# tanwanirahul/surreal

Hardware: AMD Instinct MI355X
Metric: PPO learner env-steps/sec/node (GAE+update) at 1/2/4/8 GPUs; % HBM roofline (higher is better)
Workload: dtype f32; 1 GPU; C3: synthetic PPO learner batch, reference PPO defaults (LSTM 100, horizon 5, heads 300x200, n_step 25, adapt, z-filter, 10/10 epochs), SawyerLift state dims (obs 42, act 8), 1024 segments split over 1 GPU(s) (1024 per GPU); segments_per_gpu=1024, n_step=25, env_steps_per_learn_per_gpu=25600, global_segments=1024, parallelism=single, epochs_run_last=10, ppo_mode=adapt, launch=hipGraph replay

## Files before the change

### include/surreal_mi.h

```cpp
#ifndef SURREAL_MI_H
#define SURREAL_MI_H

#include <stdint.h>

#ifdef __cplusplus
extern "C" {
#endif

#define SMI_OK            0
#define SMI_E_ARG        -1
#define SMI_E_NOFIT      -2
#define SMI_E_LAUNCH     -3

int         smi_version(void);
const char* smi_last_error(void);

const char* smi_last_launch(void);

int64_t smi_workspace_bytes(void);
int     smi_set_workspace(void* dev_ptr, int64_t bytes);
typedef struct smi_context smi_context;
smi_context* smi_context_create(void* workspace, int64_t bytes);
int          smi_context_make_current(smi_context* ctx);
int          smi_context_destroy(smi_context* ctx);
// ... 223 lines not shown
int64_t smi_ppo_rnn_xbuf_floats(int obs_dim, int rnn_hidden, int h1, int h2, int act_dim,
                                int critic_h1, int critic_h2, int pix_c, int pix_h, int pix_w,
                                int cnn_feat, int rnn_layer);
int64_t smi_lstm_param_count(int in_dim, int hidden);
int smi_ppo_rnn_phase(const smi_ppo_rnn_args* args, int phase, int epoch, void* stream);

int smi_lstm_forward(const float* xproj, const float* w_hh, const float* b_hh,
                     const float* h0, const float* c0, int S, int B, int H,
                     float* hbuf, float* cbuf, float* gates_act, void* stream);
int smi_lstm_backward(const float* dh, const float* gates_act, const float* cbuf,
                      const float* w_hh, int S, int B, int H, float* dgates, void* stream);
int smi_lstm_forward_x(const float* x, int64_t ldx, int din, const float* w_ih,
                       const float* b_ih, const float* w_hh, const float* b_hh,
                       const float* h0, const float* c0, int S, int B, int H, float* hbuf,
                       float* cbuf, float* gates_act, float* xproj_scratch, void* stream);

int64_t smi_cnn_param_count(int C, int H, int W, int F);
int64_t smi_cnn_scratch_bytes(int64_t rows, int C, int H, int W, int F);
int smi_cnn_backward_prefetch(int C, int H, int W);
int smi_cnn_forward(const float* params, const uint8_t* pix, const uint8_t* pix_next, int64_t B,
                    int64_t T, int64_t rows, int C, int H, int W, int F, float* a1, float* a2,
                    float* feat, int64_t ldf, void* stream);
int smi_cnn_backward(const float* params, const uint8_t* pix, const uint8_t* pix_next, int64_t B,
                     int64_t T, int64_t rows, int C, int H, int W, int F, const float* a1,
                     const float* a2, const float* dz, int64_t lddz, float* grad, void* scratch,
                     int64_t scratch_bytes, void* stream);

int smi_zfilter_accumulate(const float* sum_in, const float* sumsq_in, int dim, float rows,
                           float* running_sum, float* running_sumsq, float* count,
                           void* stream);
// ... 113 lines not shown
```

### surreal_amd/_lib.py

```python
import contextlib
import threading
import ctypes
import gc
import os

import torch

HERE = os.path.dirname(os.path.abspath(__file__))
_VARIANT = os.environ.get('SMI_LIB_VARIANT')
LIB_PATH = os.path.join(HERE, 'libsurreal_mi.so' if not _VARIANT else f'libsurreal_mi_{_VARIANT}.so')

c_int, c_i64, c_f32, c_f64, c_vp = ctypes.c_int, ctypes.c_int64, ctypes.c_float, ctypes.c_double, ctypes.c_void_p
P = ctypes.c_void_p

HYP_CLIP_EPS, HYP_BETA, HYP_LR_ACTOR, HYP_LR_CRITIC, HYP_CLIP_LO, HYP_CLIP_HI, HYP_COUNT = range(7)
ST_NAMES = ['_surr_loss', '_clip_surr_loss', '_kl_loss_adapt', '_entropy', '_pol_kl',
            'grad_norm_actor', '_val_loss', '_val_explained_var', 'grad_norm_critic',
            '_avg_return_targ', '_avg_log_sig', '_avg_behave_likelihood', '_avg_is_weight',
            '_ref_behave_diff', 'epochs_run', '_pol_kl_adapt']
ST_COUNT = len(ST_NAMES)
ST = {n: i for i, n in enumerate(ST_NAMES)}


class PPOArgs(ctypes.Structure):
# ... 172 lines not shown
    'smi_clock_probe': (c_int, [P, ctypes.c_longlong, P, P]),
    'smi_clock_probe_stop': (c_int, [P, c_int, P]),
    'smi_ppo_rnn_scratch_bytes': (c_i64, [c_int] * 15),
    'smi_ppo_rnn_xbuf_floats': (c_i64, [c_int] * 12),
    'smi_cnn_param_count': (c_i64, [c_int] * 4),
    'smi_cnn_scratch_bytes': (c_i64, [c_i64] + [c_int] * 4),
    'smi_cnn_backward_prefetch': (c_int, [c_int] * 3),
    'smi_cnn_forward': (c_int, [P, P, P, c_i64, c_i64, c_i64] + [c_int] * 4 + [P, P, P, c_i64, P]),
    'smi_cnn_backward': (c_int, [P, P, P, c_i64, c_i64, c_i64] + [c_int] * 4 +
                         [P, P, P, c_i64, P, P, c_i64, P]),
    'smi_ppo_rnn_phase': (c_int, [ctypes.POINTER(RNNArgs), c_int, c_int, P]),
    'smi_lstm_forward': (c_int, [P, P, P, P, P, c_int, c_int, c_int, P, P, P, P]),
    'smi_lstm_backward': (c_int, [P, P, P, P, c_int, c_int, c_int, P, P]),
    'smi_lstm_forward_x': (c_int, [P, c_i64, c_int, P, P, P, P, P, P, c_int, c_int, c_int,
                                   P, P, P, P, P]),
}

_lib = None


def lib():
    global _lib
    if _lib is None:
        if not os.path.exists(LIB_PATH):
            raise RuntimeError('libsurreal_mi.so not built: run `python -c "import __graft_entry__ as '
                               'g; g.build()"` (no CPU fallback exists)')
        L = ctypes.CDLL(LIB_PATH)
        for name, (res, args) in _SIGS.items():
            fn = getattr(L, name)
            fn.restype = res
# ... 87 lines not shown
```

### surreal_amd/csrc/capi.hip

```cpp
#include <stdio.h>
#include <string.h>
#include <atomic>
#include "smi_device.hpp"
#include "smi_internal.hpp"
#include "rnn_layout.hpp"

namespace smi {

static thread_local char g_err[512] = "";
static thread_local const char* g_last_launch = "";

int set_error(int code, const char* msg) {
  snprintf(g_err, sizeof(g_err), "%s", msg);
  return code;
}

int check_launch(const char* what) {
  g_last_launch = what;
  const hipError_t e = hipGetLastError();
  if (e != hipSuccess) {
    snprintf(g_err, sizeof(g_err), "%s: %s", what, hipGetErrorString(e));
    return -(int)e;
  }
  return SMI_OK;
// ... 789 lines not shown
                       float* gates_act, float* xproj_scratch, void* stream) {
  REQUIRE(x && w_ih && b_ih && w_hh && b_hh && h0 && c0 && hbuf && S >= 0 && B >= 0 && H >= 1 &&
          din >= 1 && ldx >= din, "lstm_forward_x: bad args");
  const hipStream_t st = SMI_STREAM(stream);
  const int rf = launch_lstm_fwd_x(x, ldx, din, w_ih, b_ih, w_hh, b_hh, h0, c0, S, B, H, hbuf, cbuf,
                                   gates_act, st, nullptr, 0);
  if (rf != SMI_E_NOFIT) return rf;
  REQUIRE(xproj_scratch, "lstm_forward_x: the unfused form needs xproj_scratch [S][B][4H]");
  const int rc = launch_linear_fwd(x, ldx, S * B, din, w_ih, din, b_ih, 4 * H, ACT_NONE,
                                   xproj_scratch, 4 * H, st, nullptr);
  if (rc) return rc;
  return launch_lstm_fwd(xproj_scratch, w_hh, b_hh, h0, c0, S, B, H, hbuf, cbuf, gates_act, st,
                         nullptr);
}

int smi_lstm_backward(const float* dh, const float* gates_act, const float* cbuf,
                      const float* w_hh, int S, int B, int H, float* dgates, void* stream) {
  REQUIRE(dh && gates_act && cbuf && w_hh && dgates && S >= 0 && B >= 0 && H >= 1,
          "lstm_backward: bad args");
  return launch_lstm_bwd(dh, gates_act, cbuf, w_hh, S, B, H, dgates, SMI_STREAM(stream), nullptr);
}

}
```

### surreal_amd/csrc/lstm_mfma.hip

```cpp
#include "smi_device.hpp"
#include "smi_internal.hpp"
#include "lstm_cell.hpp"

namespace smi {

constexpr int LR = 16;
#ifdef SMI_PROF
__device__ unsigned long long g_lstm_ticks[8];
#endif

__host__ __device__ inline int lstm_ld(int k) {
  int l = round4(k);
  if ((l & 7) != 4) l += 4;
  return l;
}

__host__ __device__ inline int lstm_q(int K) { return (((K + 3) >> 2) + 3) & ~3; }

constexpr int MAXUT = 4;
__global__ void __launch_bounds__(kWG)
lstm_fwd_kernel(LstmFwdArgs a) {
  if (a.skip && a.skip[0] != 0) return;
  const int keepS = a.keep > 0 ? a.keep : a.S;
  extern __shared__ __attribute__((aligned(16))) float sm[];
// ... 252 lines not shown
__device__ __forceinline__ void load_row_v(const float* r, int n, float* dst) {
  static_assert(N % 4 == 0 && (V == 4 || V == 2), "vector rows");
#pragma unroll
  for (int k = 0; k < N; k += V) {
    const float* src = k < n ? r + k : g_lstm_zero4;
    if constexpr (V == 4) {
      const float4 v = *reinterpret_cast<const float4*>(src);
      dst[k] = v.x; dst[k + 1] = v.y; dst[k + 2] = v.z; dst[k + 3] = v.w;
    } else {
      const float2 v = *reinterpret_cast<const float2*>(src);
      dst[k] = v.x; dst[k + 1] = v.y;
    }
  }
}

template <int KP, int KX, bool VF = false>
__global__ void __launch_bounds__(kWG8)
lstm_fwd_r4_kernel(LstmFwdArgs a) {
  if (a.skip && a.skip[0] != 0) return;
  LSTM_T0();
  const int keepS = a.keep > 0 ? a.keep : a.S;
  constexpr int KXS = KX > 0 ? KX : 8;
  __shared__ __attribute__((aligned(16))) float hS[2][LR4 * KP];
  __shared__ __attribute__((aligned(16))) float xS[2][LR4 * KXS];
  __shared__ float pre[LR4][4 * KP];
  const int H = a.H, B = a.B, G4 = 4 * H;
  const int tid = threadIdx.x, lane = tid & 63, wave = tid >> 6;
  const int r0 = blockIdx.x * LR4;
  const int64_t BH = (int64_t)B * H;
  const int col = wave * 64 + lane;
  const bool cact = wave * 64 < G4;
  const int colc = col < G4 ? col : G4 - 1;
  float w[KP];
  float wx[KXS];
  float bh = a.b_hh[colc];
  if constexpr (KX > 0) bh += a.b_ih[colc];
  if constexpr (VF) {
    load_row_v<KP, 4>(a.w_hh + (int64_t)colc * H, H, w);
    if constexpr (KX > 0) load_row_v<KX, 2>(a.w_ih + (int64_t)colc * a.din, a.din, wx);
  } else {
    load_row<KP>(a.w_hh + (int64_t)colc * H, H, w);
    if constexpr (KX > 0) load_row<KX>(a.w_ih + (int64_t)colc * a.din, a.din, wx);
  }
  const int xr = tid / KXS, xk = tid - (tid / KXS) * KXS;
  const bool xown = KX > 0 && tid < LR4 * KXS;
  const int64_t xoff0 = (int64_t)min(r0 + xr, B - 1) * a.ldx + min(xk, a.din - 1);
  const bool xval = xk < a.din;
  auto xload = [&](int t) -> float { return a.x[(int64_t)t * B * a.ldx + xoff0]; };
  float xnext = 0.f, x0 = 0.f;
  if constexpr (KX > 0) {
    x0 = xload(0);
    xnext = xload(a.S > 1 ? 1 : 0);
// ... 237 lines not shown
    __syncthreads();
  }
}

static int device_cus() {
  static int cus = 0;
  if (!cus) {
    int dev = 0;
    (void)hipGetDevice(&dev);
    if (hipDeviceGetAttribute(&cus, hipDeviceAttributeMultiprocessorCount, dev) != hipSuccess || cus < 1)
      cus = 256;
  }
  return cus;
}
static bool lstm_valu(int B, int H) { return H >= 1 && H <= 128 && B <= device_cus(); }

#ifdef SMI_PROF
extern "C" int smi_lstm_phase_ticks(unsigned long long* out ) {
  if (hipMemcpyFromSymbol(out, HIP_SYMBOL(g_lstm_ticks), sizeof(g_lstm_ticks)) != hipSuccess)
    return SMI_E_LAUNCH;
  static const unsigned long long zero[8] = {0, 0, 0, 0, 0, 0, 0, 0};
  return hipMemcpyToSymbol(HIP_SYMBOL(g_lstm_ticks), zero, sizeof(zero)) == hipSuccess ? SMI_OK
                                                                                        : SMI_E_LAUNCH;
}
#endif

int64_t lstm_fwd_lds(int H) { return (int64_t)2 * LR * lstm_ld(4 * lstm_q(H)) * 4; }
int64_t lstm_bwd_lds(int H) { return (int64_t)2 * LR * lstm_ld(4 * H) * 4; }

static bool r4_vf(const LstmFwdArgs& a, bool fused_x) {
  auto al = [](const void* p, uintptr_t m) { return (reinterpret_cast<uintptr_t>(p) & m) == 0; };
  if (a.H % 4 != 0 || !al(a.w_hh, 15)) return false;
  return !fused_x || (a.din % 2 == 0 && a.din >= 2 && al(a.w_ih, 7));
}

int launch_lstm_fwd(const float* xproj, const float* w_hh, const float* b_hh, const float* h0,
                    const float* c0, int S, int B, int H, float* hbuf, float* cbuf, float* gates,
                    hipStream_t st, const int* skip, int keep) {
  if (B <= 0 || S < 0) return SMI_OK;
  if (H < 1 || H > 256) return set_error(SMI_E_ARG, "lstm: hidden size must be in [1, 256]");
  LstmFwdArgs a{xproj, w_hh, b_hh, h0, c0, S, B, H, hbuf, cbuf, gates, skip};
  a.keep = keep;
  const int kslot = ktime_begin(st);
  struct End { int s; hipStream_t st; double f;
               ~End() { ktime_end(s, KT_LSTM_FWD, f, st); } } end_{kslot, st, 8.0 * B * H * (double)H * S};
  if (lstm_valu(B, H)) return check_launch(lstm_v_fwd(a, 0, st));
  if (H <= 128) {
    const dim3 g4((B + LR4 - 1) / LR4);
    const bool vf = r4_vf(a, false);
#define SMI_R4F(KP_)                                                                        \
    do {                                                                                    \
      if (vf) {                                                                             \
        hipLaunchKernelGGL((lstm_fwd_r4_kernel<KP_, 0, true>), g4, dim3(kWG8), 0, st, a);   \
        return check_launch("lstm_fwd_r4_kernel<" #KP_ ",0,vf>");                           \
      } else {                                                                              \
        hipLaunchKernelGGL((lstm_fwd_r4_kernel<KP_, 0>), g4, dim3(kWG8), 0, st, a);         \
        return check_launch("lstm_fwd_r4_kernel<" #KP_ ",0>");                              \
      }                                                                                     \
    } while (0)
    if (H <= 32) SMI_R4F(32);
    else if (H <= 64) SMI_R4F(64);
    else if (H <= 104) SMI_R4F(104);
    else SMI_R4F(128);
#undef SMI_R4F
  }
  const size_t lds = (size_t)lstm_fwd_lds(H);
  const dim3 grid((B + LR - 1) / LR);
  allow_lds(lstm_fwd_kernel, lds);
  hipLaunchKernelGGL(lstm_fwd_kernel, grid, dim3(kWG), lds, st, a);
  return check_launch("lstm_fwd_kernel<4>");
}

int launch_lstm_fwd_x(const float* x, int64_t ldx, int din, const float* w_ih, const float* b_ih,
                      const float* w_hh, const float* b_hh, const float* h0, const float* c0,
                      int S, int B, int H, float* hbuf, float* cbuf, float* gates,
                      hipStream_t st, const int* skip, int keep) {
  if (B <= 0 || S <= 0) return SMI_OK;
  if (din < 1 || din > 64 || H < 1 || H > 104) return SMI_E_NOFIT;
  const bool valu = lstm_valu(B, H);
  if (valu && lstm_fwd_v_lds(S, din <= 48 ? 48 : 64, (4 * H + 63) & ~63) > kVxMax)
    return SMI_E_NOFIT;
  LstmFwdArgs a{nullptr, w_hh, b_hh, h0, c0, S, B, H, hbuf, cbuf, gates, skip,
                x, ldx, din, w_ih, b_ih, keep};
  const int kslot = ktime_begin(st);
  struct End { int s; hipStream_t st; double f;
               ~End() { ktime_end(s, KT_LSTM_FWD, f, st); } } end_{
      kslot, st, 8.0 * B * H * (double)(H + din) * S};
  if (valu) return check_launch(lstm_v_fwd(a, din <= 48 ? 48 : 64, st));
  const dim3 g4((B + LR4 - 1) / LR4);
  const bool vf = r4_vf(a, true);
#define SMI_R4X(KP_, KX_)                                                                     \
  do {                                                                                        \
    if (vf) {                                                                                 \
      hipLaunchKernelGGL((lstm_fwd_r4_kernel<KP_, KX_, true>), g4, dim3(kWG8), 0, st, a);     \
      return check_launch("lstm_fwd_r4_kernel<" #KP_ "," #KX_ ",vf>");                        \
    } else {                                                                                  \
      hipLaunchKernelGGL((lstm_fwd_r4_kernel<KP_, KX_>), g4, dim3(kWG8), 0, st, a);           \
      return check_launch("lstm_fwd_r4_kernel<" #KP_ "," #KX_ ">");                           \
    }                                                                                         \
  } while (0)
  if (din <= 48) {
    if (H <= 64) SMI_R4X(64, 48);
    else SMI_R4X(104, 48);
  } else {
    if (H <= 64) SMI_R4X(64, 64);
    else SMI_R4X(104, 64);
  }
#undef SMI_R4X
// ... 64 lines not shown
```

### surreal_amd/csrc/ppo_rnn.hip

```cpp
#include "smi_device.hpp"
#include "smi_internal.hpp"
#include "dw_plan.hpp"
#include "pol_rows.hpp"
#include "lstm_cell.hpp"
#include "rnn_layout.hpp"
#include "rnn_kernels.hpp"

namespace smi {

struct Head {
  const float* P; MlpLayout L; int in, h1, h2, out, tanh_out;
};

static bool head_fused(const Head& h, const float* X, int64_t ldx) {
  return head_fused_ok(h.in, ldx, h.h1, h.h2, h.out, X, h.P + h.L.fW1, h.P + h.L.fW2,
                       h.P + h.L.fW3);
}

struct HeadFwdOpts {
  const int* skip = nullptr;
  float* wT = nullptr;
  bool keep_act = true;
  const float* vret = nullptr;
  float* vgrad = nullptr;
// ... 55 lines not shown
  RC_CHECK(launch_linear_bwd_dx(dZ, h.out, M, h.out, h.P + L.fW3, h.h2, h.h2, HA2, h.h2, dH2,
                                h.h2, st, skip));
  RC_CHECK(launch_linear_bwd_dw(dH2, h.h2, M, h.h2, HA1, h.h1, h.h1, G + L.fW2, h.h1, G + L.fb2,
                                0, st, skip));
  RC_CHECK(launch_linear_bwd_dx(dH2, h.h2, M, h.h2, h.P + L.fW2, h.h1, h.h1, HA1, h.h1, dH1,
                                h.h1, st, skip));
  RC_CHECK(launch_linear_bwd_dw(dH1, h.h1, M, h.h1, X, ldx, h.in, G + L.fW1, h.in, G + L.fb1, 0,
                                st, skip));
  if (dxn <= 0) return SMI_OK;
  return launch_linear_bwd_dx(dH1, h.h1, M, h.h1, h.P + L.fW1 + dx0, h.in, dxn, dxmask, ldm, dXout,
                              dxn, st, skip);
}

static int lstm_forward(const RnnDims& d, const float* P, const float* X, int S, const float* h0,
                        const float* c0, const RnnScratch& s, bool keep, hipStream_t st,
                        const int* skip, int keep_steps = 0) {
  const int64_t BH = (int64_t)d.B * d.H;
  for (int l = 0; l < d.L; ++l) {
    const LstmP lp = lstm_layer(d, P, l);
    const float* Xl = l == 0 ? X : hbuf_of(d, s, l - 1) + BH;
    const int64_t ldx = l == 0 ? d.ldx : d.H;
    const int din = l == 0 ? d.Din : d.H;
    float* hb = hbuf_of(d, s, l);
    float* cb = keep ? cbuf_of(d, s, l) : nullptr;
    float* gt = keep ? gates_of(d, s, l) : nullptr;
    const int rf = launch_lstm_fwd_x(Xl, ldx, din, lp.Wih, lp.bih, lp.Whh, lp.bhh, h0 + l * BH,
                                     c0 + l * BH, S, d.B, d.H, hb, cb, gt, st, skip, keep_steps);
    if (rf == SMI_E_NOFIT) {
      const int64_t rows = (int64_t)S * d.B;
      RC_CHECK(launch_linear_fwd(Xl, ldx, (int)rows, din, lp.Wih, din, lp.bih, d.G4, ACT_NONE,
                                 s.xproj, d.G4, st, skip));
      RC_CHECK(launch_lstm_fwd(s.xproj, lp.Whh, lp.bhh, h0 + l * BH, c0 + l * BH, S, d.B, d.H, hb,
                               cb, gt, st, skip, keep_steps));
    } else if (rf) {
      return rf;
    }
  }
  return SMI_OK;
}

static int lstm_backward(const RnnDims& d, const float* P, float* G, const RnnScratch& s,
                         hipStream_t st, const int* skip) {
  const int64_t BH = (int64_t)d.B * d.H;
  const int M = (int)d.NE;
  for (int l = d.L - 1; l >= 0; --l) {
    const LstmP lp = lstm_layer(d, P, l);
    float* dg = dgates_of(d, s, l);
    float* hb = hbuf_of(d, s, l);
// ... 83 lines not shown
  const int rf = dw_group_flush(st);
  return rc ? rc : rf;
}

static float c_loglik_of(int A) { return (float)(0.5 * log(2.0 * 3.141592653589793) * (double)A); }
static float c_entropy_of(int A) {
  return (float)(0.5 * log(2.0 * 3.141592653589793 * 2.718281828459045) * (double)A);
}

int64_t ppo_rnn_scratch_bytes(int B, int T, int Hz, int D, int H, int L, int h1, int h2, int A, int c1,
                              int c2, int pc, int ph, int pw, int F) {
  return 4 * rnn_scratch(rnn_dims(B, T, Hz, D, H, h1, h2, A, c1, c2, pc, ph, pw, F, L), nullptr)
                 .total_floats;
}

static PolRowArgs pol_rows(const smi_ppo_rnn_args& a, const RnnDims& d, const RnnScratch& s) {
  PolRowArgs p{};
  p.B = d.B; p.T = d.T; p.E = d.E; p.A = d.A; p.mode = a.mode;
  p.mu = s.OUT; p.lv = a.actor + d.LA.flv; p.refmu = s.refmu; p.ref_lv = a.ref_actor + d.LA.flv;
  p.actions = a.actions; p.behave = a.behave; p.adv = s.adv; p.ret = s.ret;
  p.rowin = s.rowin; p.ret_tm = s.ret_tm;
  p.moments = a.moments; p.norm_adv = a.norm_adv; p.c_ll = c_loglik_of(d.A);
  p.hyper = a.hyper; p.skip = s.ci + CI_STOP;
  p.part = s.part; p.dz = s.dOUT; p.lvpart = s.lvpart; p.cf = s.cf;
  return p;
}

struct Ctx {
  const smi_ppo_rnn_args& a;
  RnnDims d;
  RnnScratch s;
  const int* stop;
  LstmP lm;
  const float* cnn;
  Head actor, critic;
  float *gA, *gC;
  int64_t NEg;
  hipStream_t st;
};

static Ctx make_ctx(const smi_ppo_rnn_args& a, hipStream_t st) {
  const RnnDims d = rnn_dims(a.B, a.T, a.horizon, a.obs_dim, a.rnn_hidden, a.h1, a.h2, a.act_dim,
                             a.critic_h1, a.critic_h2, a.pix_c, a.pix_h, a.pix_w, a.cnn_feat,
                             a.rnn_layer);
  const RnnScratch s = rnn_scratch(d, a.scratch);
  return Ctx{a, d, s, s.ci + CI_STOP, lstm_params(a.lstm, d.Din, d.H), a.lstm + d.nL,
             Head{a.actor, d.LA, d.Hin, d.h1, d.h2, d.A, 1},
             Head{a.critic, d.LC, d.Hin, d.c1, d.c2, 1, 0},
             a.xbuf, a.xbuf + d.nA_head + d.nS, (int64_t)d.E * a.B_global, st};
}

struct Rules {
  const smi_ppo_rnn_args& a;
  const RnnDims& d;
  const RnnScratch& s;
  const Head& actor;

  bool fused_clip_norm() const {
    if (a.B_global != a.B || d.F != 0 || d.L > 3 || fault() != 0) return false;
    const bool heads = dw_group_takes(d.h1, d.Hin + 1) && dw_group_takes(d.h2, d.h1 + 1) &&
                       dw_group_takes(d.A, d.h2 + 1) && dw_group_takes(d.c1, d.Hin + 1) &&
                       dw_group_takes(d.c2, d.c1 + 1) && dw_group_takes(1, d.c2 + 1);
    const bool stem = d.H == 0 || (dw_group_takes(d.G4, d.ldx + d.H + 1) &&
                                   (d.L == 1 || dw_group_takes(d.G4, d.H + d.H + 1)));
// ... 50 lines not shown
  RC_CHECK(cnn_features(a, d, c.cnn, d.S1, s.Xz, nullptr, s, st, nullptr));
  if (r.gae_prep_dual()) {
    RC_CHECK(launch_zf_tmajor(a.obs, a.obs_next, d.B, d.T, d.E, d.D, a.use_zf, a.rzf_sum,
                              a.rzf_sumsq, a.rzf_count, a.zf_eps, s.Xr, d.ldx, st, 0,
                              d.F == 0));
    const LstmP lc = lstm_layer(d, a.lstm, 0), lr = lstm_layer(d, a.ref_lstm, 0);
    LstmFwdArgs g0{nullptr, lc.Whh, lc.bhh, a.h0, a.c0, d.S1, d.B, d.H, hbuf_of(d, s, 0),
                   cbuf_of(d, s, 0), gates_of(d, s, 0), nullptr, s.Xz, d.ldx, d.Din, lc.Wih,
                   lc.bih, d.E};
    LstmFwdArgs g1{nullptr, lr.Whh, lr.bhh, a.h0, a.c0, d.E, d.B, d.H, s.hbufR, nullptr, nullptr,
                   nullptr, s.Xr, d.ldx, d.Din, lr.Wih, lr.bih, 0};
    RC_CHECK(launch_lstm_fwd_x_dual(g0, g1, st));
  } else if (d.H > 0) {
    RC_CHECK(lstm_forward(d, a.lstm, s.Xz, d.S1, a.h0, a.c0, s, true, st, nullptr, d.E));
  }
  RC_CHECK(head_fwd(c.critic, head_in(d, s, s.Xz), d.Hld, d.NG, s.HA1, s.HA2, s.OUT, st,
                    fwd_only()));
  RC_CHECK(launch_tmajor_to_bmajor(s.OUT, d.S1, d.B, s.values, s.ci, s.cf, st));
  int np = 0;
  kt = ktime_begin(st);
  RC_CHECK(launch_gae_windows(s.values, nullptr, a.rewards, a.dones, d.B, d.T, d.Hz, a.gamma_tab,
                              a.lam_tab, a.gamma, a.gamma_H, s.adv, s.ret, s.gaepart, &np, st));
  ktime_end(kt, KT_GAE, (double)d.B * (8.0 * d.T + 4.0 * d.S1 + 8.0 * d.E), st);
  return launch_reduce_partials(s.gaepart, np, 2, a.moments, nullptr, a.moments + 2,
                                (double)d.NE, st);
}

static int phase_prep(const Ctx& c, const Rules& r) {
  const smi_ppo_rnn_args& a = c.a;
  const RnnDims& d = c.d;
// ... 12 lines not shown
  }
  const Head ref{a.ref_actor, d.LA, d.Hin, d.h1, d.h2, d.A, 1};
  return head_fwd(ref, head_in(d, sp, X), d.Hld, d.NE, sp.HA1, sp.HA2, s.refmu, st, fwd_only());
}

static int phase_policy_fwd(const Ctx& c, const Rules& r, int e) {
  const smi_ppo_rnn_args& a = c.a;
  const RnnDims& d = c.d;
  const RnnScratch& s = c.s;
  hipStream_t st = c.st;
  if (e == 0) RC_CHECK(launch_row_pack(d.A, d.NE, pol_rows(a, d, s), s.rowin, s.ret_tm, st));
  if (e == 0 && (a.adv_out || a.ret_out))
    RC_CHECK(launch_adv_export(pol_rows(a, d, s), d.NE, a.adv_out, a.ret_out, st));
  RC_CHECK(cnn_features(a, d, c.cnn, d.E, s.Xz, s.A1, s, st, c.stop));
  if (d.H > 0 && e > 0)
    RC_CHECK(lstm_forward(d, a.lstm, s.Xz, d.E, a.h0, a.c0, s, true, st, c.stop));
  PolRowArgs p = pol_rows(a, d, s);
  p.invN = (float)(1.0 / (double)c.NEg);
  const bool bwd_next = e < a.epoch_policy;
  HeadFwdOpts o;
  o.skip = c.stop;
  o.wT = bwd_next ? s.wT : nullptr;
  o.keep_act = bwd_next;
  RC_CHECK(head_fwd(c.actor, head_in(d, s, s.Xz), d.Hld, d.NE, s.HA1, s.HA2, s.OUT, st, o));
  const int nb = r.pol_stats_nb();
  RC_CHECK(launch_pol_stats(a.mode == 0, nb, p, st));
  if (r.fused_decide(e)) return SMI_OK;
  if (a.B_global == a.B)
    return launch_reduce_decide(s.part, nb, decide_args(c, e), c.stop, st);
  return launch_reduce_partials(s.part, nb, PS_N, a.pstat, c.stop, nullptr, 0.0, st);
}
// ... 34 lines not shown
  const smi_ppo_rnn_args& a = c.a;
  const RnnDims& d = c.d;
  const int64_t nS = !policy && fault() == SMI_FAULT_CRITIC_STEM_OMIT ? 0 : d.nS;
  const int64_t n_head = policy ? d.nA_head : d.nC_head;
  const int g = grid_of(n_head + nS, 1024);
  const bool fn = r.fused_clip_norm();
  const bool clip = policy ? a.clip_actor_grad : a.clip_critic_grad;
  const float max_norm = policy ? a.actor_max_norm : a.critic_max_norm;
  float* norm_out = a.stats + (policy ? SMI_ST_GRAD_NORM_ACTOR : SMI_ST_GRAD_NORM_CRITIC);
  AdamSplitArgs aa{policy ? a.actor : a.critic, n_head, a.lstm, nS, policy ? c.gA : c.gC,
                   policy ? a.actor_m : a.critic_m, policy ? a.actor_v : a.critic_v,
                   policy ? a.actor_step : a.critic_step,
                   a.hyper + (policy ? SMI_HYP_LR_ACTOR : SMI_HYP_LR_CRITIC), a.beta1, a.beta2,
                   a.adam_eps, policy ? a.actor_wd : a.critic_wd, clip ? max_norm : 0.f,
                   c.s.part, g, policy ? c.stop : nullptr, clip ? norm_out : nullptr, nullptr,
                   fn ? c.s.ci + CI_NP : nullptr};
  return launch_adam_split(aa, g, fn ? nullptr : c.s.part, policy ? c.s.ci + CI_RUNS : nullptr,
                           c.st);
}

static int phase_policy_apply(const Ctx& c, const Rules& r, int e) {
  if (fault() == SMI_FAULT_POLICY_EPOCH_SHORT && e == c.a.epoch_policy - 1) return SMI_OK;
  return adam_apply(c, r, true);
}

static int phase_value_grad(const Ctx& c, const Rules& r, int e) {
  const smi_ppo_rnn_args& a = c.a;
  const RnnDims& d = c.d;
  const RnnScratch& s = c.s;
  hipStream_t st = c.st;
  if (e > 0) {
    RC_CHECK(cnn_features(a, d, c.cnn, d.E, s.Xz, s.A1, s, st, nullptr));
    if (d.H > 0)
      RC_CHECK(lstm_forward(d, a.lstm, s.Xz, d.E, a.h0, a.c0, s, true, st, nullptr));
  }
  const bool last = e == a.epoch_baseline - 1;
  const float vscale = (float)(2.0 / (double)c.NEg);
  bool vdone = false;
  const bool vstats = r.vstats(e);
  HeadFwdOpts o;
  o.wT = s.wT;
  o.vret = last && !vstats ? nullptr : s.ret_tm;
  o.vgrad = last && !vstats ? nullptr : s.dOUT;
  o.vscale = vscale;
  o.vpart = vstats ? s.part : nullptr;
  o.vdone = &vdone;
  RC_CHECK(head_fwd(c.critic, head_in(d, s, s.Xz), d.Hld, d.NE, s.HA1, s.HA2, s.OUT, st, o));
  int nb = rnn_nblk((d.NE + 3) / 4, kRowNT);
  if (vdone && vstats) nb = head_bwd_blocks(d.NE);
// ... 58 lines not shown
```

### surreal_amd/csrc/ppo_rnn_kernels.hip

```cpp
#include <type_traits>
#include "smi_device.hpp"
#include "smi_internal.hpp"
#include "pol_rows.hpp"
#include "rnn_kernels.hpp"

namespace smi {

constexpr int kZfRows = 8;
__global__ void __launch_bounds__(kWG)
zf_tmajor_kernel(const float* __restrict__ obs, const float* __restrict__ obs_next, int B, int T,
                 int S, int D, int use_zf, const float* zs, const float* zq, const float* zc,
                 float eps, float* __restrict__ out, int ldo) {
  if (D <= 0) return;
  extern __shared__ __attribute__((aligned(16))) float sm[];
  float* zm = sm;
  float* zd = sm + round4(D);
  if (use_zf) zfilter_colstats(zs, zq, zc, eps, D, zm, zd);
  __syncthreads();
  const int lane = threadIdx.x & 63;
  const int nrows = S * B;
  const int w0 = blockIdx.x * (kWG / 64) + (threadIdx.x >> 6), nw = gridDim.x * (kWG / 64);
  float m0 = 0.f, d0 = 1.f, m1 = 0.f, d1 = 1.f;
  if (use_zf) {
    if (lane < D) { m0 = zm[lane]; d0 = zd[lane]; }
// ... 779 lines not shown
  const float w2 = (float)(1.0 - (double)a.beta2);
  for (int64_t i = i_first; i < n; i += (int64_t)gridDim.x * kWG) {
    const bool fst = i == i_first;
    float* pp = fst ? pf : i < a.n0 ? a.p0 + i : a.p1 + (i - a.n0);
    float g = (fst ? gf : a.g[i]) * coef;
    float p = fst ? pvf : *pp;
    if (a.wd != 0.f) g = g + a.wd * p;
    float mi = fst ? mf : a.m[i], vi = fst ? vf : a.v[i];
    mi = mi + w1 * (g - mi);
    vi = vi * a.beta2 + (w2 * g) * g;
    const float denom = sqrtf(vi) / bc2_sqrt + a.eps;
    *pp = p + (-step_size) * (mi / denom);
    a.m[i] = mi;
    a.v[i] = vi;
  }
}

__global__ void __launch_bounds__(kWG)
sumsq_part_kernel(const float* __restrict__ g, int64_t n, double* part, const int* skip,
                  int* step, int* runs) {
  if (skip && skip[0] != 0) return;
  if (blockIdx.x == 0 && threadIdx.x == 0) {
    step[0] += 1;
    if (runs) runs[0] += 1;
  }
  __shared__ double scr[kNW];
  double s = 0.0;
  for (int64_t i = (int64_t)blockIdx.x * kWG + threadIdx.x; i < n; i += (int64_t)gridDim.x * kWG) {
    const double v = (double)g[i];
    s += v * v;
// ... 231 lines not shown
```

### surreal_amd/csrc/rnn_kernels.hpp

```cpp
#pragma once
#include "smi_internal.hpp"
#include "pol_rows.hpp"

namespace smi {

enum { FS_SE = 0, FS_D, FS_D2, FS_R, FS_R2, FS_Z = 5 };

inline int rnn_nblk(int64_t rows, int nt = kWG) {
  const int64_t cap = (int64_t)1024 * kWG / nt;
  const int64_t b = (rows + nt - 1) / nt;
  return (int)(b < cap ? (b < 1 ? 1 : b) : cap);
}
constexpr int kRowNT = 64;
inline int grid_of(int64_t n, int cap = 1024) {
  int64_t g = (n + kWG - 1) / kWG;
  if (g < 1) g = 1;
  return (int)(g < cap ? g : cap);
}

int launch_zf_tmajor(const float* obs, const float* obs_next, int B, int T, int S, int D,
                     int use_zf, const float* zs, const float* zq, const float* zc, float eps,
                     float* out, int ldo, hipStream_t st, int form = 0, bool pad_ok = false);
int launch_tmajor_to_bmajor(const float* vt, int S, int B, float* v, int* ci, float* cf,
                            hipStream_t st);
// ... 9 lines not shown
int launch_policy_decide(const DecideArgs& da, hipStream_t st);
int launch_reduce_decide(const double* part, int nb, const DecideArgs& da, const int* skip,
                         hipStream_t st);
int launch_value_rows(const float* V, const float* ret_tm, int B, int E, float invN2, float* dV,
                      double* part, int nb, hipStream_t st);
int launch_obs_iter_colsum(const float* obs, int B, int T, int E, int D, double* part, int nb,
                           hipStream_t st);

struct AdamSplitArgs {
  float* p0; int64_t n0; float* p1; int64_t n1;
  const float* g; float* m; float* v;
  int* step; const float* lr_ptr; float beta1, beta2, eps, wd, max_norm;
  const double* part; int np;
  const int* skip; float* norm_out; int* runs;
  const int* np_dev;
};
int launch_adam_split(const AdamSplitArgs& a, int grid, double* sumsq_part, int* runs,
                      hipStream_t st);

struct FinalArgs {
  const double* fs; int D; int64_t N; const float* lv; int A; int clip_critic;
  float* zs; float* zq; float* zc; int use_zf;
  float* stats; const int* ci; float* kl_record; int* kl_count; int kl_capacity; int Ep;
};
int launch_rnn_final(const FinalArgs& a, hipStream_t st);

}
```

### surreal_amd/csrc/rnn_layout.hpp

```cpp
#pragma once
#include "smi_shapes.hpp"

namespace smi {

struct RnnDims {
  int B, T, Hz, E, S1, D, H, G4, A, h1, h2, c1, c2;
  int L;
  int64_t nL0, nLk;
  int F, Din;
  int Hin;
  int ldx;
  int Hld;
  int64_t NE, NG;
  int64_t nA_head, nC_head, nL, nCnn, nS;
  MlpLayout LA, LC;
  CnnGeom G;
};

inline RnnDims rnn_dims(int B, int T, int Hz, int D, int H, int h1, int h2, int A, int c1, int c2,
                        int pc = 0, int ph = 0, int pw = 0, int F = 0, int L = 1) {
  RnnDims d;
  d.L = L > 1 ? L : 1;
  d.F = F > 0 ? F : 0; d.Din = D + d.F;
  d.G = cnn_geom(pc, ph, pw, d.F);
// ... 11 lines not shown
  d.nLk = H > 0 ? (int64_t)8 * H * H + 8 * (int64_t)H : 0;
  d.nL = d.nL0 + (d.L - 1) * d.nLk;
  d.nS = d.nL + d.nCnn;
  return d;
}

struct RnnScratch {
  float *Xz, *Xr, *xproj, *hbuf, *cbuf, *gates, *HA1, *HA2, *OUT, *dOUT, *dH1, *dH2, *dh, *dgates;
  float *xprojR, *hbufR, *HA1R, *HA2R, *A2R;
  float *wT;
  float *values, *adv, *ret, *refmu, *lvpart;
  float *rowin, *ret_tm;
  float *A1, *A2, *dA2, *dF, *cpart;
  double *part, *gaepart;
  int* ci; float* cf;
  int64_t total_floats;
};

inline int64_t al64(int64_t n) { return (n + 63) & ~(int64_t)63; }
inline int64_t part_doubles(const RnnDims& d) {
  const int64_t v = 5 * (int64_t)head_bwd_blocks(d.NE);
  return v > 65536 ? v : 65536;
}
inline RnnScratch rnn_scratch(const RnnDims& d, void* base) {
  RnnScratch s{};
  float* p = static_cast<float*>(base);
  int64_t o = 0;
  auto take = [&](int64_t n) { float* r = p ? p + o : nullptr; o += al64(n); return r; };
  const int hmax1 = d.h1 > d.c1 ? d.h1 : d.c1, hmax2 = d.h2 > d.c2 ? d.h2 : d.c2;
  s.Xz = take(d.NG * d.ldx);
  s.Xr = take(d.NE * d.ldx);
  s.xproj = take(d.NG * d.G4);
  s.hbuf = take((int64_t)d.L * (d.S1 + 1) * d.B * d.H);
  s.cbuf = take((int64_t)d.L * (d.E + 1) * d.B * d.H);
  s.gates = take((int64_t)d.L * d.NE * d.G4);
  s.HA1 = take(d.NG * hmax1);
  s.HA2 = take(d.NG * hmax2);
  s.OUT = take(d.NG * (d.A > 1 ? d.A : 1));
  s.dOUT = take(d.NE * (d.A > 1 ? d.A : 1));
  s.dH1 = take(d.NE * hmax1);
  s.dH2 = take(d.NE * hmax2);
  s.dh = take(d.NE * d.H);
  s.dgates = take((int64_t)d.L * d.NE * d.G4);
  s.values = take((int64_t)d.B * d.S1);
  s.adv = take(d.NE);
  s.ret = take(d.NE);
  s.refmu = take(d.NE * d.A);
// ... 56 lines not shown
```

### surreal_amd/csrc/smi_internal.hpp

```cpp
#pragma once
#include <hip/hip_runtime.h>
#include <stdint.h>
#include "../../include/surreal_mi.h"
#include "smi_shapes.hpp"

namespace smi {

int set_error(int code, const char* msg);

enum { KT_GEMM_FWD = 0, KT_GEMM_DX, KT_GEMM_DW, KT_GEMM_REDUCE, KT_LSTM_FWD, KT_LSTM_BWD,
       KT_CNN_FWD, KT_CNN_BWD,
       KT_GAE, KT_POLICY_STATS, KT_POLICY_GRAD, KT_VALUE_ROWS, KT_ADAM, KT_ZF_TMAJOR,
       KT_COUNT };
bool ktime_on();
int ktime_begin(hipStream_t st);
void ktime_end(int slot, int cls, double flops, hipStream_t st);
int64_t smi_workspace_floats();
float* workspace_f32(int64_t nfloats);
void workspace_reserve(int64_t nfloats);
int launch_linear_fwd(const float* X, int64_t ldx, int M, int K, const float* W, int64_t ldw,
                      const float* b, int N, int act, float* Y, int64_t ldy, hipStream_t st,
                      const int* skip = nullptr);
int launch_linear_bwd_dx(const float* dY, int64_t ldg, int M, int N, const float* W, int64_t ldw,
                         int K, const float* mask, int64_t ldm, float* dX, int64_t lddx,
// ... 69 lines not shown
                      const float* gtab, const float* ltab, float gamma, float gamma_T,
                      float* values, float* adv, float* ret, hipStream_t stream);
int gae_windows_max_partials(int64_t B, int T);
int launch_gae_windows(const float* values, float* values_masked, const float* rewards, const float* dones, int64_t B,
                       int T, int H, const float* gtab, const float* ltab, float gamma,
                       float gamma_H, float* adv, float* ret, double* partials,
                       int* n_partials, hipStream_t stream);
int launch_ppo_fused(const smi_ppo_args* args, hipStream_t stream);
int64_t ppo_fused_max_params();
int64_t ppo_xbuf_floats(int D, int H1, int H2, int A, int cH1, int cH2, int mode);
int launch_ppo_epoch_grad(const smi_ppo_args* args, int epoch, hipStream_t stream);
int launch_ppo_epoch_apply(const smi_ppo_args* args, int epoch, hipStream_t stream);

int64_t ppo_rnn_scratch_bytes(int B, int T, int Hz, int D, int H, int L, int h1, int h2, int A, int c1,
                              int c2, int pc, int ph, int pw, int F);
int ppo_rnn_phase(const smi_ppo_rnn_args& a, int phase, int e, hipStream_t st);
int launch_lstm_fwd(const float* xproj, const float* w_hh, const float* b_hh, const float* h0,
                    const float* c0, int S, int B, int H, float* hbuf, float* cbuf, float* gates,
                    hipStream_t st, const int* skip, int keep = 0);
int launch_lstm_fwd_x(const float* x, int64_t ldx, int din, const float* w_ih, const float* b_ih,
                      const float* w_hh, const float* b_hh, const float* h0, const float* c0,
                      int S, int B, int H, float* hbuf, float* cbuf, float* gates,
                      hipStream_t st, const int* skip, int keep = 0);
int launch_lstm_bwd(const float* dh, const float* gates, const float* cbuf, const float* w_hh,
                    int S, int B, int H, float* dgates, hipStream_t st, const int* skip);

}

#include "smi_launch.hpp"
```

Measured before the change: 3.940 million env-steps/s.

## Keep a transposed LSTM weight image for coalesced recurrent-kernel weight loads

Adds a k-major (transposed) copy of the LSTM input and recurrent weights, stored in unused xproj scratch space. It is built after the first forward and refreshed inside the Adam update kernel. The r4 forward LSTM kernel gains an IMG variant that reads weight columns from this image, so per-thread weight loads walk along columns instead of strided rows. The cost is an extra transpose pass in the optimizer step and tighter coupling between the scratch layout and the parameter update.

```diff
diff --git a/include/surreal_mi.h b/include/surreal_mi.h
--- a/include/surreal_mi.h
+++ b/include/surreal_mi.h
@@ -261,6 +261,15 @@
                        const float* b_ih, const float* w_hh, const float* b_hh,
                        const float* h0, const float* c0, int S, int B, int H, float* hbuf,
                        float* cbuf, float* gates_act, float* xproj_scratch, void* stream);
+int smi_lstm_weight_image(const float* w_ih, const float* w_hh, int din, int H, float* image,
+                          void* stream);
+int smi_lstm_forward_x_image(const float* x, int64_t ldx, int din, const float* w_ih,
+                             const float* b_ih, const float* image, const float* b_hh,
+                             const float* h0, const float* c0, int S, int B, int H, float* hbuf,
+                             float* cbuf, float* gates_act, float* xproj_scratch, void* stream);
+int64_t smi_ppo_rnn_wimage_offset(int B, int T, int horizon, int obs_dim, int rnn_hidden,
+                                  int h1, int h2, int act_dim, int critic_h1, int critic_h2,
+                                  int pix_c, int pix_h, int pix_w, int cnn_feat, int rnn_layer);
 
 int64_t smi_cnn_param_count(int C, int H, int W, int F);
 int64_t smi_cnn_scratch_bytes(int64_t rows, int C, int H, int W, int F);
diff --git a/surreal_amd/_lib.py b/surreal_amd/_lib.py
--- a/surreal_amd/_lib.py
+++ b/surreal_amd/_lib.py
@@ -210,6 +210,10 @@
     'smi_lstm_backward': (c_int, [P, P, P, P, c_int, c_int, c_int, P, P]),
     'smi_lstm_forward_x': (c_int, [P, c_i64, c_int, P, P, P, P, P, P, c_int, c_int, c_int,
                                    P, P, P, P, P]),
+    'smi_lstm_weight_image': (c_int, [P, P, c_int, c_int, P, P]),
+    'smi_lstm_forward_x_image': (c_int, [P, c_i64, c_int, P, P, P, P, P, P, c_int, c_int, c_int,
+                                         P, P, P, P, P]),
+    'smi_ppo_rnn_wimage_offset': (c_i64, [c_int] * 15),
 }
 
 _lib = None
diff --git a/surreal_amd/csrc/capi.hip b/surreal_amd/csrc/capi.hip
--- a/surreal_amd/csrc/capi.hip
+++ b/surreal_amd/csrc/capi.hip
@@ -827,6 +827,41 @@
                          nullptr);
 }
 
+int64_t smi_ppo_rnn_wimage_offset(int B, int T, int horizon, int obs_dim, int rnn_hidden, int h1,
+                                  int h2, int act_dim, int critic_h1, int critic_h2, int pix_c,
+                                  int pix_h, int pix_w, int cnn_feat, int rnn_layer) {
+  return ppo_rnn_wimage_offset(B, T, horizon, obs_dim, rnn_hidden, rnn_layer, h1, h2, act_dim,
+                               critic_h1, critic_h2, pix_c, pix_h, pix_w, cnn_feat);
+}
+
+int smi_lstm_weight_image(const float* w_ih, const float* w_hh, int din, int H, float* image,
+                          void* stream) {
+  REQUIRE(w_ih && w_hh && image, "lstm_weight_image: bad args");
+  return launch_lstm_weight_image(w_ih, w_hh, din, H, image, SMI_STREAM(stream));
+}
+
+int smi_lstm_forward_x_image(const float* x, int64_t ldx, int din, const float* w_ih,
+                             const float* b_ih, const float* image, const float* b_hh,
+                             const float* h0, const float* c0, int S, int B, int H, float* hbuf,
+                             float* cbuf, float* gates_act, float* xproj_scratch, void* stream) {
+  REQUIRE(x && b_ih && image && b_hh && h0 && c0 && hbuf && S >= 0 && B >= 0 && H >= 1 &&
+          din >= 1 && ldx >= din, "lstm_forward_x_image: bad args");
+  if (S == 0 || B == 0) return SMI_OK;
+  if (!lstm_fwd_image_ok(B, H)) return SMI_E_NOFIT;
+  const hipStream_t st = SMI_STREAM(stream);
+  const float* w_hhT = image + (int64_t)4 * H * din;
+  const int rf = launch_lstm_fwd_x(x, ldx, din, image, b_ih, w_hhT, b_hh, h0, c0, S, B, H, hbuf,
+                                   cbuf, gates_act, st, nullptr, 0, true);
+  if (rf != SMI_E_NOFIT) return rf;
+  REQUIRE(w_ih && xproj_scratch,
+          "lstm_forward_x_image: the unfused form needs w_ih and xproj_scratch [S][B][4H]");
+  const int rc = launch_linear_fwd(x, ldx, S * B, din, w_ih, din, b_ih, 4 * H, ACT_NONE,
+                                   xproj_scratch, 4 * H, st, nullptr);
+  if (rc) return rc;
+  return launch_lstm_fwd(xproj_scratch, w_hhT, b_hh, h0, c0, S, B, H, hbuf, cbuf, gates_act, st,
+                         nullptr, 0, true);
+}
+
 int smi_lstm_backward(const float* dh, const float* gates_act, const float* cbuf,
                       const float* w_hh, int S, int B, int H, float* dgates, void* stream) {
   REQUIRE(dh && gates_act && cbuf && w_hh && dgates && S >= 0 && B >= 0 && H >= 1,
diff --git a/surreal_amd/csrc/lstm_mfma.hip b/surreal_amd/csrc/lstm_mfma.hip
--- a/surreal_amd/csrc/lstm_mfma.hip
+++ b/surreal_amd/csrc/lstm_mfma.hip
@@ -290,7 +290,17 @@
   }
 }
 
-template <int KP, int KX, bool VF = false>
+template <int N>
+__device__ __forceinline__ void load_col(const float* t, int n, int ld, uint32_t zoff, int col,
+                                         float* dst) {
+#pragma unroll
+  for (int k = 0; k < N; ++k) {
+    const uint32_t row = k < n ? (uint32_t)(k * ld) : zoff;
+    dst[k] = t[row + (uint32_t)col];
+  }
+}
+
+template <int KP, int KX, bool VF = false, bool IMG = false>
 __global__ void __launch_bounds__(kWG8)
 lstm_fwd_r4_kernel(LstmFwdArgs a) {
   if (a.skip && a.skip[0] != 0) return;
@@ -311,7 +321,10 @@
   float wx[KXS];
   float bh = a.b_hh[colc];
   if constexpr (KX > 0) bh += a.b_ih[colc];
-  if constexpr (VF) {
+  if constexpr (IMG) {
+    load_col<KP>(a.w_hh, H, G4, (uint32_t)(H * G4), colc, w);
+    if constexpr (KX > 0) load_col<KX>(a.w_ih, a.din, G4, (uint32_t)((a.din + H) * G4), colc, wx);
+  } else if constexpr (VF) {
     load_row_v<KP, 4>(a.w_hh + (int64_t)colc * H, H, w);
     if constexpr (KX > 0) load_row_v<KX, 2>(a.w_ih + (int64_t)colc * a.din, a.din, wx);
   } else {
@@ -579,6 +592,34 @@
   return cus;
 }
 static bool lstm_valu(int B, int H) { return H >= 1 && H <= 128 && B <= device_cus(); }
+bool lstm_fwd_image_ok(int B, int H) { return H >= 1 && H <= 128 && B >= 1 && !lstm_valu(B, H); }
+
+__global__ void __launch_bounds__(kWG)
+lstm_weight_image_kernel(const float* __restrict__ w_ih, const float* __restrict__ w_hh, int din,
+                         int H, float* __restrict__ image) {
+  const int G4 = 4 * H, nih = G4 * din, nw = nih + G4 * H;
+  const int o = blockIdx.x * kWG + threadIdx.x;
+  if (o >= nw + G4) return;
+  if (o < nih) {
+    const int k = o / G4, col = o - k * G4;
+    image[o] = w_ih[col * din + k];
+  } else if (o < nw) {
+    const int k = (o - nih) / G4, col = (o - nih) - k * G4;
+    image[o] = w_hh[col * H + k];
+  } else {
+    image[o] = 0.f;
+  }
+}
+
+int launch_lstm_weight_image(const float* w_ih, const float* w_hh, int din, int H, float* image,
+                             hipStream_t st) {
+  if (H < 1 || H > 128 || din < 1 || din > 4096)
+    return set_error(SMI_E_ARG, "lstm_weight_image: H must be in [1, 128], din in [1, 4096]");
+  const int n = 4 * H * (din + H + 1);
+  hipLaunchKernelGGL(lstm_weight_image_kernel, dim3((n + kWG - 1) / kWG), dim3(kWG), 0, st, w_ih,
+                     w_hh, din, H, image);
+  return check_launch("lstm_weight_image_kernel");
+}
 
 #ifdef SMI_PROF
 extern "C" int smi_lstm_phase_ticks(unsigned long long* out ) {
@@ -601,9 +642,10 @@
 
 int launch_lstm_fwd(const float* xproj, const float* w_hh, const float* b_hh, const float* h0,
                     const float* c0, int S, int B, int H, float* hbuf, float* cbuf, float* gates,
-                    hipStream_t st, const int* skip, int keep) {
+                    hipStream_t st, const int* skip, int keep, bool image) {
   if (B <= 0 || S < 0) return SMI_OK;
   if (H < 1 || H > 256) return set_error(SMI_E_ARG, "lstm: hidden size must be in [1, 256]");
+  if (image && !lstm_fwd_image_ok(B, H)) return SMI_E_NOFIT;
   LstmFwdArgs a{xproj, w_hh, b_hh, h0, c0, S, B, H, hbuf, cbuf, gates, skip};
   a.keep = keep;
   const int kslot = ktime_begin(st);
@@ -615,7 +657,11 @@
     const bool vf = r4_vf(a, false);
 #define SMI_R4F(KP_)                                                                        \
     do {                                                                                    \
-      if (vf) {                                                                             \
+      if (image) {                                                                          \
+        hipLaunchKernelGGL((lstm_fwd_r4_kernel<KP_, 0, false, true>), g4, dim3(kWG8), 0,    \
+                           st, a);                                                          \
+        return check_launch("lstm_fwd_r4_kernel<" #KP_ ",0,img>");                          \
+      } else if (vf) {                                                                      \
         hipLaunchKernelGGL((lstm_fwd_r4_kernel<KP_, 0, true>), g4, dim3(kWG8), 0, st, a);   \
         return check_launch("lstm_fwd_r4_kernel<" #KP_ ",0,vf>");                           \
       } else {                                                                              \
@@ -639,10 +685,13 @@
 int launch_lstm_fwd_x(const float* x, int64_t ldx, int din, const float* w_ih, const float* b_ih,
                       const float* w_hh, const float* b_hh, const float* h0, const float* c0,
                       int S, int B, int H, float* hbuf, float* cbuf, float* gates,
-                      hipStream_t st, const int* skip, int keep) {
+                      hipStream_t st, const int* skip, int keep, bool image) {
   if (B <= 0 || S <= 0) return SMI_OK;
-  if (din < 1 || din > 64 || H < 1 || H > 104) return SMI_E_NOFIT;
+  if (!lstm_fwd_x_fuses(din, H)) return SMI_E_NOFIT;
   const bool valu = lstm_valu(B, H);
+  if (image && valu) return SMI_E_NOFIT;
+  if (image && w_hh != w_ih + (int64_t)4 * H * din)
+    return set_error(SMI_E_ARG, "lstm: W_hhT must follow W_ihT in the weight image");
   if (valu && lstm_fwd_v_lds(S, din <= 48 ? 48 : 64, (4 * H + 63) & ~63) > kVxMax)
     return SMI_E_NOFIT;
   LstmFwdArgs a{nullptr, w_hh, b_hh, h0, c0, S, B, H, hbuf, cbuf, gates, skip,
@@ -656,7 +705,11 @@
   const bool vf = r4_vf(a, true);
 #define SMI_R4X(KP_, KX_)                                                                     \
   do {                                                                                        \
-    if (vf) {                                                                                 \
+    if (image) {                                                                              \
+      hipLaunchKernelGGL((lstm_fwd_r4_kernel<KP_, KX_, false, true>), g4, dim3(kWG8), 0, st,  \
+                         a);                                                                  \
+      return check_launch("lstm_fwd_r4_kernel<" #KP_ "," #KX_ ",img>");                       \
+    } else if (vf) {                                                                          \
       hipLaunchKernelGGL((lstm_fwd_r4_kernel<KP_, KX_, true>), g4, dim3(kWG8), 0, st, a);     \
       return check_launch("lstm_fwd_r4_kernel<" #KP_ "," #KX_ ",vf>");                        \
     } else {                                                                                  \
diff --git a/surreal_amd/csrc/ppo_rnn.hip b/surreal_amd/csrc/ppo_rnn.hip
--- a/surreal_amd/csrc/ppo_rnn.hip
+++ b/surreal_amd/csrc/ppo_rnn.hip
@@ -93,24 +93,28 @@
 
 static int lstm_forward(const RnnDims& d, const float* P, const float* X, int S, const float* h0,
                         const float* c0, const RnnScratch& s, bool keep, hipStream_t st,
-                        const int* skip, int keep_steps = 0) {
+                        const int* skip, int keep_steps = 0, const float* wimg = nullptr) {
   const int64_t BH = (int64_t)d.B * d.H;
   for (int l = 0; l < d.L; ++l) {
     const LstmP lp = lstm_layer(d, P, l);
+    const bool img = wimg && l == 0;
+    const float* rWih = img ? wimg : lp.Wih;
+    const float* rWhh = img ? wimg + (int64_t)d.G4 * d.Din : lp.Whh;
     const float* Xl = l == 0 ? X : hbuf_of(d, s, l - 1) + BH;
     const int64_t ldx = l == 0 ? d.ldx : d.H;
     const int din = l == 0 ? d.Din : d.H;
     float* hb = hbuf_of(d, s, l);
     float* cb = keep ? cbuf_of(d, s, l) : nullptr;
     float* gt = keep ? gates_of(d, s, l) : nullptr;
-    const int rf = launch_lstm_fwd_x(Xl, ldx, din, lp.Wih, lp.bih, lp.Whh, lp.bhh, h0 + l * BH,
-                                     c0 + l * BH, S, d.B, d.H, hb, cb, gt, st, skip, keep_steps);
+    const int rf = launch_lstm_fwd_x(Xl, ldx, din, rWih, lp.bih, rWhh, lp.bhh, h0 + l * BH,
+                                     c0 + l * BH, S, d.B, d.H, hb, cb, gt, st, skip, keep_steps,
+                                     img);
     if (rf == SMI_E_NOFIT) {
       const int64_t rows = (int64_t)S * d.B;
       RC_CHECK(launch_linear_fwd(Xl, ldx, (int)rows, din, lp.Wih, din, lp.bih, d.G4, ACT_NONE,
                                  s.xproj, d.G4, st, skip));
-      RC_CHECK(launch_lstm_fwd(s.xproj, lp.Whh, lp.bhh, h0 + l * BH, c0 + l * BH, S, d.B, d.H, hb,
-                               cb, gt, st, skip, keep_steps));
+      RC_CHECK(launch_lstm_fwd(s.xproj, rWhh, lp.bhh, h0 + l * BH, c0 + l * BH, S, d.B, d.H, hb,
+                               cb, gt, st, skip, keep_steps, img));
     } else if (rf) {
       return rf;
     }
@@ -224,6 +228,12 @@
                  .total_floats;
 }
 
+int64_t ppo_rnn_wimage_offset(int B, int T, int Hz, int D, int H, int L, int h1, int h2, int A, int c1,
+                              int c2, int pc, int ph, int pw, int F) {
+  return rnn_scratch(rnn_dims(B, T, Hz, D, H, h1, h2, A, c1, c2, pc, ph, pw, F, L), nullptr)
+      .wimg_off;
+}
+
 static PolRowArgs pol_rows(const smi_ppo_rnn_args& a, const RnnDims& d, const RnnScratch& s) {
   PolRowArgs p{};
   p.B = d.B; p.T = d.T; p.E = d.E; p.A = d.A; p.mode = a.mode;
@@ -247,6 +257,7 @@
   float *gA, *gC;
   int64_t NEg;
   hipStream_t st;
+  float* wimg;
 };
 
 static Ctx make_ctx(const smi_ppo_rnn_args& a, hipStream_t st) {
@@ -257,7 +268,8 @@
   return Ctx{a, d, s, s.ci + CI_STOP, lstm_params(a.lstm, d.Din, d.H), a.lstm + d.nL,
              Head{a.actor, d.LA, d.Hin, d.h1, d.h2, d.A, 1},
              Head{a.critic, d.LC, d.Hin, d.c1, d.c2, 1, 0},
-             a.xbuf, a.xbuf + d.nA_head + d.nS, (int64_t)d.E * a.B_global, st};
+             a.xbuf, a.xbuf + d.nA_head + d.nS, (int64_t)d.E * a.B_global, st,
+             s.wimg && lstm_fwd_image_ok(d.B, d.H) ? s.wimg : nullptr};
 }
 
 struct Rules {
@@ -338,6 +350,7 @@
   } else if (d.H > 0) {
     RC_CHECK(lstm_forward(d, a.lstm, s.Xz, d.S1, a.h0, a.c0, s, true, st, nullptr, d.E));
   }
+  if (c.wimg) RC_CHECK(launch_lstm_weight_image(c.lm.Wih, c.lm.Whh, d.Din, d.H, c.wimg, st));
   RC_CHECK(head_fwd(c.critic, head_in(d, s, s.Xz), d.Hld, d.NG, s.HA1, s.HA2, s.OUT, st,
                     fwd_only()));
   RC_CHECK(launch_tmajor_to_bmajor(s.OUT, d.S1, d.B, s.values, s.ci, s.cf, st));
@@ -380,7 +393,7 @@
     RC_CHECK(launch_adv_export(pol_rows(a, d, s), d.NE, a.adv_out, a.ret_out, st));
   RC_CHECK(cnn_features(a, d, c.cnn, d.E, s.Xz, s.A1, s, st, c.stop));
   if (d.H > 0 && e > 0)
-    RC_CHECK(lstm_forward(d, a.lstm, s.Xz, d.E, a.h0, a.c0, s, true, st, c.stop));
+    RC_CHECK(lstm_forward(d, a.lstm, s.Xz, d.E, a.h0, a.c0, s, true, st, c.stop, 0, c.wimg));
   PolRowArgs p = pol_rows(a, d, s);
   p.invN = (float)(1.0 / (double)c.NEg);
   const bool bwd_next = e < a.epoch_policy;
@@ -445,7 +458,8 @@
                    a.hyper + (policy ? SMI_HYP_LR_ACTOR : SMI_HYP_LR_CRITIC), a.beta1, a.beta2,
                    a.adam_eps, policy ? a.actor_wd : a.critic_wd, clip ? max_norm : 0.f,
                    c.s.part, g, policy ? c.stop : nullptr, clip ? norm_out : nullptr, nullptr,
-                   fn ? c.s.ci + CI_NP : nullptr};
+                   fn ? c.s.ci + CI_NP : nullptr, c.wimg, d.Din, d.H,
+                   lstm_fwd_x_fuses(d.Din, d.H) ? 1 : 0};
   return launch_adam_split(aa, g, fn ? nullptr : c.s.part, policy ? c.s.ci + CI_RUNS : nullptr,
                            c.st);
 }
@@ -463,7 +477,7 @@
   if (e > 0) {
     RC_CHECK(cnn_features(a, d, c.cnn, d.E, s.Xz, s.A1, s, st, nullptr));
     if (d.H > 0)
-      RC_CHECK(lstm_forward(d, a.lstm, s.Xz, d.E, a.h0, a.c0, s, true, st, nullptr));
+      RC_CHECK(lstm_forward(d, a.lstm, s.Xz, d.E, a.h0, a.c0, s, true, st, nullptr, 0, c.wimg));
   }
   const bool last = e == a.epoch_baseline - 1;
   const float vscale = (float)(2.0 / (double)c.NEg);
diff --git a/surreal_amd/csrc/ppo_rnn_kernels.hip b/surreal_amd/csrc/ppo_rnn_kernels.hip
--- a/surreal_amd/csrc/ppo_rnn_kernels.hip
+++ b/surreal_amd/csrc/ppo_rnn_kernels.hip
@@ -817,6 +817,21 @@
     a.m[i] = mi;
     a.v[i] = vi;
   }
+  if (a.wimg) {
+    const int G4 = 4 * a.wH, nih = G4 * a.wdin, nw = nih + G4 * a.wH;
+    for (int64_t i = i_first; i < n; i += (int64_t)gridDim.x * kWG) {
+      const int64_t j = i - a.n0;
+      if (j < (a.wih ? 0 : nih) || j >= nw) continue;
+      const float pn = a.p1[j];
+      if (j < nih) {
+        const int r = (int)j / a.wdin, k = (int)j - r * a.wdin;
+        a.wimg[k * G4 + r] = pn;
+      } else {
+        const int jh = (int)j - nih, r = jh / a.wH, k = jh - r * a.wH;
+        a.wimg[nih + k * G4 + r] = pn;
+      }
+    }
+  }
 }
 
 __global__ void __launch_bounds__(kWG)
diff --git a/surreal_amd/csrc/rnn_kernels.hpp b/surreal_amd/csrc/rnn_kernels.hpp
--- a/surreal_amd/csrc/rnn_kernels.hpp
+++ b/surreal_amd/csrc/rnn_kernels.hpp
@@ -47,6 +47,7 @@
   const double* part; int np;
   const int* skip; float* norm_out; int* runs;
   const int* np_dev;
+  float* wimg; int wdin, wH, wih;
 };
 int launch_adam_split(const AdamSplitArgs& a, int grid, double* sumsq_part, int* runs,
                       hipStream_t st);
diff --git a/surreal_amd/csrc/rnn_layout.hpp b/surreal_amd/csrc/rnn_layout.hpp
--- a/surreal_amd/csrc/rnn_layout.hpp
+++ b/surreal_amd/csrc/rnn_layout.hpp
@@ -49,10 +49,19 @@
   float *A1, *A2, *dA2, *dF, *cpart;
   double *part, *gaepart;
   int* ci; float* cf;
+  float* wimg;
+  int64_t wimg_off;
   int64_t total_floats;
 };
 
 inline int64_t al64(int64_t n) { return (n + 63) & ~(int64_t)63; }
+inline int64_t wimg_floats(const RnnDims& d) {
+  return d.L == 1 && d.H >= 1 && d.H <= 128 ? (int64_t)d.G4 * (d.Din + d.H + 1) : 0;
+}
+inline int64_t wimg_in_xproj(const RnnDims& d) {
+  const int64_t n = wimg_floats(d), at = al64(d.NE * d.G4);
+  return n > 0 && at + n <= d.NG * d.G4 ? at : -1;
+}
 inline int64_t part_doubles(const RnnDims& d) {
   const int64_t v = 5 * (int64_t)head_bwd_blocks(d.NE);
   return v > 65536 ? v : 65536;
@@ -65,7 +74,9 @@
   const int hmax1 = d.h1 > d.c1 ? d.h1 : d.c1, hmax2 = d.h2 > d.c2 ? d.h2 : d.c2;
   s.Xz = take(d.NG * d.ldx);
   s.Xr = take(d.NE * d.ldx);
+  s.wimg_off = wimg_in_xproj(d) >= 0 ? o + wimg_in_xproj(d) : -1;
   s.xproj = take(d.NG * d.G4);
+  s.wimg = s.xproj && s.wimg_off >= 0 ? p + s.wimg_off : nullptr;
   s.hbuf = take((int64_t)d.L * (d.S1 + 1) * d.B * d.H);
   s.cbuf = take((int64_t)d.L * (d.E + 1) * d.B * d.H);
   s.gates = take((int64_t)d.L * d.NE * d.G4);
diff --git a/surreal_amd/csrc/smi_internal.hpp b/surreal_amd/csrc/smi_internal.hpp
--- a/surreal_amd/csrc/smi_internal.hpp
+++ b/surreal_amd/csrc/smi_internal.hpp
@@ -107,14 +107,20 @@
 
 int64_t ppo_rnn_scratch_bytes(int B, int T, int Hz, int D, int H, int L, int h1, int h2, int A, int c1,
                               int c2, int pc, int ph, int pw, int F);
+int64_t ppo_rnn_wimage_offset(int B, int T, int Hz, int D, int H, int L, int h1, int h2, int A, int c1,
+                              int c2, int pc, int ph, int pw, int F);
 int ppo_rnn_phase(const smi_ppo_rnn_args& a, int phase, int e, hipStream_t st);
 int launch_lstm_fwd(const float* xproj, const float* w_hh, const float* b_hh, const float* h0,
                     const float* c0, int S, int B, int H, float* hbuf, float* cbuf, float* gates,
-                    hipStream_t st, const int* skip, int keep = 0);
+                    hipStream_t st, const int* skip, int keep = 0, bool image = false);
+bool lstm_fwd_image_ok(int B, int H);
+inline bool lstm_fwd_x_fuses(int din, int H) { return din >= 1 && din <= 64 && H >= 1 && H <= 104; }
+int launch_lstm_weight_image(const float* w_ih, const float* w_hh, int din, int H, float* image,
+                             hipStream_t st);
 int launch_lstm_fwd_x(const float* x, int64_t ldx, int din, const float* w_ih, const float* b_ih,
                       const float* w_hh, const float* b_hh, const float* h0, const float* c0,
                       int S, int B, int H, float* hbuf, float* cbuf, float* gates,
-                      hipStream_t st, const int* skip, int keep = 0);
+                      hipStream_t st, const int* skip, int keep = 0, bool image = false);
 int launch_lstm_bwd(const float* dh, const float* gates, const float* cbuf, const float* w_hh,
                     int S, int B, int H, float* dgates, hipStream_t st, const int* skip);
 
```

Result: faster. 3.985 million env-steps/s, median of 6 (+1.2%).
